# baggepinnen/LPVSpectral.jl

Hardware: NVIDIA B200
Metric: windowed LS spectra/sec (higher is better)
Workload: dtype f64

## Files before the change

### lpvspectral.jl_b200/csrc/api.cu

```cuda
#include <math.h>
#include <stdarg.h>
#include <stdlib.h>
#include <stdio.h>
#include <string.h>

#include <algorithm>

#include "ctx.h"

namespace lpvs {

int fail(lpvs_ctx* c, int code, const char* fmt, ...) {
    char buf[512];
    va_list ap;
    va_start(ap, fmt);
    vsnprintf(buf, sizeof buf, fmt, ap);
    va_end(ap);
    if (c) c->err = buf;
    return code;
}

void* ws_raw(lpvs_ctx* c, int slot, size_t bytes) {
    DevBuf& b = c->buf[slot];
    if (bytes == 0) bytes = 16;
// ... 140 lines not shown
    if (i >= count) return;
    double s = accumulate ? out[i] : 0.0;
    for (int p = 0; p < nparts; p++) s += parts[(long long)p * stride + i];
    out[i] = s;
}

__global__ void k_check_finite(const double* __restrict__ v, long long n, int* flag) {
    bool bad = false;
    for (long long i = (long long)blockIdx.x * blockDim.x + threadIdx.x; i < n; i += (long long)gridDim.x * blockDim.x)
        bad |= !isfinite(v[i]);
    if (bad) atomicOr(flag, 1);
}

__global__ void k_first_nonfinite_channel(const double* __restrict__ Y, long long ldY, long long N, int* out) {
    const int ch = blockIdx.y;
    bool bad = false;
    for (long long i = (long long)blockIdx.x * blockDim.x + threadIdx.x; i < N; i += (long long)gridDim.x * blockDim.x)
        bad |= !isfinite(Y[ch * ldY + i]);
    if (bad) atomicMin(out, ch);
}

__global__ void k_jitter_ridge(const double* __restrict__ maxdiag, double ridge, double scale, double* __restrict__ out) {
    out[0] = fmax(ridge, scale * maxdiag[0]);
}

__global__ void k_merge_windows(const double* __restrict__ pieces, long long K, int n, int hop, long long N,
                                double* __restrict__ out) {
    const long long s = (long long)blockIdx.x * blockDim.x + threadIdx.x;
    if (s >= N) return;
    long long k0 = s >= n ? (s - n + hop) / hop : 0;
    long long k1 = s / hop;
    if (k1 > K - 1) k1 = K - 1;
    double acc = 0.0;
    long long cnt = 0;
    for (long long k = k0; k <= k1; k++) {
        acc += pieces[k * n + (s - k * hop)];
        cnt++;
    }
    out[s] = acc / (double)(cnt > 0 ? cnt : 1);
}

__global__ void k_x_to_complex(const double* __restrict__ X, int Np, int Nf, int zero_first, int nrhs,
                               double* __restrict__ out) {
    int k = blockIdx.x * blockDim.x + threadIdx.x;
    if (k >= Nf) return;
    int pc = (k >> 6) * 128 + (k & 63);
    for (int r = 0; r < nrhs; r++) {
        double re = X[(long long)r * Np + pc];
        double im = (zero_first && k == 0) ? 0.0 : X[(long long)r * Np + pc + 64];
        out[((long long)r * Nf + k) * 2] = re;
        out[((long long)r * Nf + k) * 2 + 1] = im;
    }
}

__device__ __forceinline__ int ref_to_internal(int j, int Nf, int zero_first) {
    if (j < Nf) return (j >> 6) * 128 + (j & 63);
    int k = j - Nf + zero_first;
    return (k >> 6) * 128 + 64 + (k & 63);
}
__global__ void k_gather_ref(const double* __restrict__ G, const double* __restrict__ B, int Np, int Nf,
                             int zero_first, int Nreg, double* __restrict__ Gout, double* __restrict__ bout) {
    int j = blockIdx.x * blockDim.x + threadIdx.x;
    int i = blockIdx.y;
    if (j >= Nreg) return;
    int pi = ref_to_internal(i, Nf, zero_first), pj = ref_to_internal(j, Nf, zero_first);
    int a = max(pi, pj), b = min(pi, pj);
    double v = G[(long long)a * Np + b];
    Gout[(long long)i * Nreg + j] = v;
    if (bout && i == 0) bout[j] = B[pj];
}
__global__ void k_scatter_ref_vec(const double* __restrict__ xin, int Nf, int zero_first, int Nreg, int Np,
                                  double* __restrict__ xout) {
    int p = blockIdx.x * blockDim.x + threadIdx.x;
    if (p >= Np) return;
    int q = p >> 7, r = p & 127, part = r >> 6, cc = q * 64 + (r & 63);
    double v = 0.0;
    if (cc < Nf && !(zero_first && part == 1 && cc == 0)) {
        int j = part == 0 ? cc : (Nf + cc - zero_first);
        v = xin[j];
    }
    xout[p] = v;
}

__global__ void k_window_accum(int kind, const double* __restrict__ X, long long strideB, int Np, int nwin, int Nf,
                               int zero_first, double* __restrict__ sums) {
    int k = blockIdx.x * blockDim.x + threadIdx.x;
    if (k >= Nf) return;
    int pc = (k >> 6) * 128 + (k & 63);
    bool noim = zero_first && k == 0;
    if (kind == LPVS_WIN_PSD) {
        double s = sums[k];
        for (int wdx = 0; wdx < nwin; wdx++) {
            const double* x = X + (long long)wdx * strideB;
            double re = x[pc], im = noim ? 0.0 : x[pc + 64];
            s = __dadd_rn(s, __dadd_rn(__dmul_rn(re, re), __dmul_rn(im, im)));
        }
        sums[k] = s;
    } else if (kind == LPVS_WIN_CSD) {
        double sr = sums[k], si = sums[Nf + k];
        for (int wdx = 0; wdx < nwin; wdx++) {
            const double* x = X + (long long)wdx * strideB;
            double ar = x[pc], ai = noim ? 0.0 : x[pc + 64];
            double br = x[Np + pc], bi = noim ? 0.0 : x[Np + pc + 64];
            sr = __dadd_rn(sr, __dadd_rn(__dmul_rn(ar, br), __dmul_rn(ai, bi)));
            si = __dadd_rn(si, __dsub_rn(__dmul_rn(ai, br), __dmul_rn(ar, bi)));
        }
        sums[k] = sr;
        sums[Nf + k] = si;
    } else {
        double syy = sums[k], suu = sums[Nf + k], sr = sums[2 * Nf + k], si = sums[3 * Nf + k];
        for (int wdx = 0; wdx < nwin; wdx++) {
            const double* x = X + (long long)wdx * strideB;
            double ar = x[pc], ai = noim ? 0.0 : x[pc + 64];
            double br = x[Np + pc], bi = noim ? 0.0 : x[Np + pc + 64];
            sr = __dadd_rn(sr, __dadd_rn(__dmul_rn(ar, br), __dmul_rn(ai, bi)));
            si = __dadd_rn(si, __dsub_rn(__dmul_rn(ai, br), __dmul_rn(ar, bi)));
            syy = __dadd_rn(syy, __dadd_rn(__dmul_rn(ar, ar), __dmul_rn(ai, ai)));
            suu = __dadd_rn(suu, __dadd_rn(__dmul_rn(br, br), __dmul_rn(bi, bi)));
        }
        sums[k] = syy;
        sums[Nf + k] = suu;
        sums[2 * Nf + k] = sr;
        sums[3 * Nf + k] = si;
    }
}

__global__ void k_window_matrix_accum(const double* __restrict__ X, long long strideB, int Np, int C, int nwin, int Nf,
                                      int zero_first, double* __restrict__ sums) {
    const long long idx = (long long)blockIdx.x * blockDim.x + threadIdx.x;
    if (idx >= (long long)Nf * C * C) return;
    const int k = (int)(idx / ((long long)C * C)), i = (int)(idx / C % C), j = (int)(idx % C);
    if (i > j) return;
    const int pc = (k >> 6) * 128 + (k & 63);
    const bool noim = zero_first && k == 0;
    double* sij = sums + 2 * (((long long)k * C + i) * C + j);
    double sr = sij[0], si = sij[1];
    for (int wdx = 0; wdx < nwin; wdx++) {
        const double* xi = X + (long long)wdx * strideB + (long long)i * Np;
        const double* xj = X + (long long)wdx * strideB + (long long)j * Np;
        const double ar = xi[pc], ai = noim ? 0.0 : xi[pc + 64];
        const double br = xj[pc], bi = noim ? 0.0 : xj[pc + 64];
        sr = __dadd_rn(sr, __dadd_rn(__dmul_rn(ar, br), __dmul_rn(ai, bi)));
        si = __dadd_rn(si, __dsub_rn(__dmul_rn(ai, br), __dmul_rn(ar, bi)));
    }
    sij[0] = sr;
    sij[1] = si;
    if (i != j) {
        double* sji = sums + 2 * (((long long)k * C + j) * C + i);
        sji[0] = sr;
        sji[1] = -si;
    }
}

void fill_basis_args(const FourierPlan& pl, GramArgs& g) {
    g.ncc = pl.Nf;
    g.nblk = pl.nblk;
    g.f = pl.d_f;
    g.wtab = pl.d_wtab;
    g.gscale = pl.dd * pl.dd;
    g.bscale = pl.dd;
    g.E = nullptr;
    g.Kt = nullptr;
    g.lpv_nf = 1;
}

static int structured_sums(lpvs_ctx* c, const FourierPlan& pl, const StructuredLayout& lay, const GramArgs& g, int nprob,
                           double2* Z) {
    double2* tab = ws<double2>(c, BUF_SANC, (size_t)lay.nrows * g.tbl_ns);
    if (!tab) return fail(c, LPVS_E_NOMEM, "out of device memory (sum tables)");
    launch_sum_tables(g.t, g.tbl_base, g.tbl_ns, pl.d_sfreq, lay.nzb, structured_layout(pl.f0, pl.Nf, 2).nzb, tab, c->st);
    SumArgs a{};
    a.t = g.t;
    a.W = g.W;
    a.y = g.y;
    a.u = g.u;
    a.w_abs = g.w_abs;
    a.start0 = g.start0;
    a.hop = g.hop;
    a.n = g.n;
    a.s_end = g.s_end;
    a.tab = tab;
    a.tbl_base = g.tbl_base;
    a.tbl_ns = g.tbl_ns;
    a.nzg = lay.nzg;
    a.nby = lay.nby;
    a.nzb = lay.nzb;
    a.Z = Z;
    a.strideZ = (long long)lay.nzb * FB;
    c->launches += 1 + launch_trig_sums(a, nprob, c->st);
    return LPVS_OK;
}
static void structured_fill(lpvs_ctx* c, const FourierPlan& pl, const StructuredLayout& lay, const double2* Z, double* G,
                            long long strideG, double* B, long long strideB, int nrhs, int nprob) {
    FillArgs fa{};
    fa.Z = Z;
    fa.strideZ = (long long)lay.nzb * FB;
    fa.zm_off = lay.zm_off;
    fa.zp_off = lay.zp_off;
    fa.zy_off[0] = lay.zy_off[0];
    fa.zy_off[1] = lay.zy_off[1];
    fa.ncc = pl.Nf;
    fa.nblk = pl.nblk;
    fa.zero_first = pl.zero_first;
    fa.gscale = pl.dd * pl.dd;
    fa.G = G;
    fa.strideG = strideG;
    c->launches += launch_gram_fill(fa, nprob, c->st);
// ... 383 lines not shown
        case LPVS_OPT_ADMM_SYMV: c->admm_symv = (int)value; break;
        case LPVS_OPT_TRSV_FLOW: c->trsv_flow = (int)value != 0; break;
        case LPVS_OPT_ADMM_M32: c->admm_m32 = (int)value != 0; break;
        case LPVS_OPT_SHARD_EXCHANGE:
            if ((int)value < 0 || (int)value > 2) return fail(c, LPVS_E_BAD_ARG, "LPVS_OPT_SHARD_EXCHANGE must be 0, 1 or 2");
            c->shard_exchange = (int)value;
            break;
        default: return fail(c, LPVS_E_BAD_ARG, "unknown option %d", key);
    }
    return LPVS_OK;
}

int lpvs_set_stream(lpvs_ctx* c, void* stream) {
    if (!c) return LPVS_E_BAD_ARG;
    Lock lk(c->mu);
    cudaSetDevice(c->device);
    cudaStreamSynchronize(c->st);
    c->st = stream ? (cudaStream_t)stream : c->own_st;
    return LPVS_OK;
}

int64_t lpvs_launch_count(const lpvs_ctx* c) { return c ? c->launches : 0; }

int lpvs_last_gram_timing(const lpvs_ctx* c, double* ms, int64_t* launches, double* flops) {
    if (!c) return LPVS_E_BAD_ARG;
    if (ms) *ms = c->gram_ms;
    if (launches) *launches = c->gram_launches;
    if (flops) *flops = c->gram_flops;
    return LPVS_OK;
}

int lpvs_last_call_ms(const lpvs_ctx* c, double* ms) {
    if (!c || !ms) return LPVS_E_BAD_ARG;
    float m = 0.f;
    if (cudaEventSynchronize(c->ev_call1) != cudaSuccess || cudaEventElapsedTime(&m, c->ev_call0, c->ev_call1) != cudaSuccess) {
        cudaGetLastError();
        return LPVS_E_CUDA;
    }
    *ms = m;
    return LPVS_OK;
}

int lpvs_dev_alloc(lpvs_ctx* c, int64_t bytes, void** dptr) {
    if (!c || !dptr) return LPVS_E_BAD_ARG;
    cudaSetDevice(c->device);
    LPVS_CU(c, cudaMalloc(dptr, (size_t)bytes));
    return LPVS_OK;
}
int lpvs_dev_free(lpvs_ctx* c, void* dptr) {
    if (!c) return LPVS_E_BAD_ARG;
    cudaSetDevice(c->device);
    cudaStreamSynchronize(c->st);
    LPVS_CU(c, cudaFree(dptr));
    return LPVS_OK;
}
int lpvs_dev_upload(lpvs_ctx* c, void* dptr, const void* hptr, int64_t bytes) {
    if (!c) return LPVS_E_BAD_ARG;
    cudaSetDevice(c->device);
    LPVS_CU(c, cudaMemcpyAsync(dptr, hptr, (size_t)bytes, cudaMemcpyHostToDevice, c->st));
    LPVS_CU(c, cudaStreamSynchronize(c->st));
    return LPVS_OK;
}
int lpvs_dev_download(lpvs_ctx* c, void* hptr, const void* dptr, int64_t bytes) {
    if (!c) return LPVS_E_BAD_ARG;
    cudaSetDevice(c->device);
    LPVS_CU(c, cudaMemcpyAsync(hptr, dptr, (size_t)bytes, cudaMemcpyDeviceToHost, c->st));
    LPVS_CU(c, cudaStreamSynchronize(c->st));
    return LPVS_OK;
}
int lpvs_release_workspace(lpvs_ctx* c) {
    if (!c) return LPVS_E_BAD_ARG;
    Lock lk(c->mu);
    cudaSetDevice(c->device);
    LPVS_CU(c, cudaStreamSynchronize(c->st));
    for (auto& b : c->buf) {
        if (b.p) cudaFree(b.p);
        b.p = nullptr;
        b.cap = 0;
    }
    return LPVS_OK;
}
int lpvs_sync(lpvs_ctx* c) {
    if (!c) return LPVS_E_BAD_ARG;
    LPVS_CU(c, cudaStreamSynchronize(c->st));
    return LPVS_OK;
}

int64_t lpvs_window_count(int64_t N, int n, int noverlap) {
    if (n <= 0) return 0;
    if (noverlap < 0) noverlap = n >> 1;
    if (noverlap >= n) return -1;
    return N >= n ? (N - n) / (n - noverlap) + 1 : 0;
}

int lpvs_gram_fourier(lpvs_ctx* c, const double* y, const double* t, int64_t N, const double* f, int Nf,
                      const double* W, double* G, double* b) {
    if (!c) return LPVS_E_BAD_ARG;
    Lock lk(c->mu);
    CallTimer call_timer(c);
    cudaSetDevice(c->device);
    if (!t || N <= 0 || !G) return fail(c, LPVS_E_BAD_ARG, "bad arguments");
    gram_timer_reset(c);
    FourierPlan pl;
    int rc = make_fourier_plan(c, f, Nf, &pl);
    if (rc) return rc;
    double *d_t, *d_y, *d_W;
    if ((rc = upload(c, BUF_T, t, N, &d_t))) return rc;
    if ((rc = upload(c, BUF_Y, y, N, &d_y))) return rc;
    if ((rc = upload(c, BUF_W, W, N, &d_W))) return rc;
    const long long Np = pl.Np;
    double* d_G = ws<double>(c, BUF_G, (size_t)Np * Np);
    double* d_B = ws<double>(c, BUF_B, (size_t)2 * Np);
    if (!d_G || !d_B) return fail(c, LPVS_E_NOMEM, "out of device memory (G)");
    if ((rc = gram_single(c, pl, d_t, d_y, nullptr, d_W, N, y ? 1 : 0, d_G, d_B))) return rc;
    double* d_out = ws<double>(c, BUF_MISC, (size_t)pl.Nreg * pl.Nreg + pl.Nreg);
    if (!d_out) return fail(c, LPVS_E_NOMEM, "out of device memory (G out)");
    dim3 grid((pl.Nreg + 127) / 128, pl.Nreg);
    k_gather_ref<<<grid, 128, 0, c->st>>>(d_G, (y && b) ? d_B : nullptr, pl.Np, pl.Nf, pl.zero_first, pl.Nreg, d_out,
                                          (y && b) ? d_out + (size_t)pl.Nreg * pl.Nreg : nullptr);
    c->launches++;
    LPVS_CU(c, cudaMemcpyAsync(G, d_out, sizeof(double) * pl.Nreg * pl.Nreg, cudaMemcpyDeviceToHost, c->st));
    if (y && b)
        LPVS_CU(c, cudaMemcpyAsync(b, d_out + (size_t)pl.Nreg * pl.Nreg, sizeof(double) * pl.Nreg,
                                   cudaMemcpyDeviceToHost, c->st));
    LPVS_CU(c, cudaStreamSynchronize(c->st));
    gram_timer_resolve(c);
    return LPVS_OK;
}

}

namespace lpvs {
int ls_solve_dev(lpvs_ctx* c, const FourierPlan& pl, const double* d_t, const double* d_y, const double* d_u,
                        const double* d_W, int64_t N, int nrhs, double ridge, bool allow_jitter, double** d_x,
                        int* info) {
    const long long Np = pl.Np;
    double* d_G = ws<double>(c, BUF_G, (size_t)Np * Np);
    double* d_B = ws<double>(c, BUF_B, (size_t)2 * Np);
    double* d_md = ws<double>(c, BUF_SUMS, 8);
    if (!d_G || !d_B || !d_md) return fail(c, LPVS_E_NOMEM, "out of device memory (G)");
    int rc;
    if (info) *info = 0;
    if (!d_W && nrhs == 1 && allow_jitter) {
        auto regram = [&]() { return gram_single(c, pl, d_t, d_y, nullptr, nullptr, N, 1, d_G, d_B); };
        if ((rc = regram())) return rc;
        OpArgs op;
        op.mode = GRAM_DIRECT;
        op.t = d_t;
        op.f = pl.d_f;
        op.dd = pl.dd;
        op.ncc = pl.Nf;
        op.zero_first = pl.zero_first;
        op.N = N;
        if ((rc = ls_solve_accurate(c, op, pl.Np, pl.zero_first, d_y, d_G, d_B, sqrt(ridge), regram, info))) return rc;
        *d_x = d_B;
        return LPVS_OK;
    }
    double* d_keep = nullptr;
    for (int attempt = 0; attempt < 2; attempt++) {
        if (attempt == 0) {
            if ((rc = gram_single(c, pl, d_t, d_y, d_u, d_W, N, nrhs, d_G, d_B))) return rc;
            if (allow_jitter) {
                d_keep = ws<double>(c, BUF_YINV, (size_t)Np * Np + 2 * Np);
                if (d_keep) {
                    LPVS_CU(c, cudaMemcpyAsync(d_keep, d_G, sizeof(double) * Np * Np, cudaMemcpyDeviceToDevice, c->st));
                    LPVS_CU(c, cudaMemcpyAsync(d_keep + Np * Np, d_B, sizeof(double) * 2 * Np, cudaMemcpyDeviceToDevice,
// ... 318 lines not shown
        double* d_G = ws<double>(c, BUF_G, (size_t)nw * Np * Np);
        double* d_B = ws<double>(c, BUF_B, (size_t)nw * 2 * Np);
        if (!d_G || !d_B) return fail(c, LPVS_E_NOMEM, "out of device memory (window batch of %d)", nw);
        GramArgs g{};
        fill_basis_args(pl, g);
        auto chain_tables = [&]() -> int {
            double2* anc = ws<double2>(c, BUF_ANC, (size_t)pl.ngroups * ns);
            double2* del = ws<double2>(c, BUF_DEL, (size_t)ns);
            if (!anc || !del) return fail(c, LPVS_E_NOMEM, "out of device memory (anchor table)");
            launch_anchor_table(d_t, s0, ns, pl.d_f, pl.nblk, pl.df, anc, del, c->st);
            c->launches++;
            g.anc = anc;
            g.del = del;
            return LPVS_OK;
        };
        if (gram_is_chain(pl.mode) && !pl.structured && (rc = chain_tables())) return rc;
        g.t = d_t;
        g.y = d_y;
        g.u = nrhs > 1 ? d_u : nullptr;
        g.W = d_W;
        g.w_abs = 0;
        g.start0 = s0;
        g.hop = hop;
        g.n = n;
        g.s_end = N;
        g.nrhs = nrhs;
        g.tbl_base = s0;
        g.tbl_ns = ns;
        g.G = d_G;
        g.strideG = Np * Np;
        g.B = d_B;
        g.strideB = 2 * Np;
        gram_timer_begin(c);
        if (pl.structured) {
            const StructuredLayout lay = structured_layout(pl.f0, Nf, nrhs);
            double2* Z = ws<double2>(c, BUF_ZSUM, (size_t)nw * lay.nzb * FB);
            if (!Z) return fail(c, LPVS_E_NOMEM, "out of device memory (window sums)");
            if ((rc = structured_sums(c, pl, lay, g, nw, Z))) return rc;
            structured_fill(c, pl, lay, Z, d_G, Np * Np, d_B, 2 * Np, nrhs, nw);
            if (pl.structured_ref && (rc = structured_correct(c, pl, g, d_G, Np * Np, d_B, 2 * Np, nrhs, nw, k_begin * hop,
                                                              (k_end - 1 - k_begin) * hop + n)))
                return rc;
            gram_timer_end(c, (double)nw * n * lay.nzb * FB * 8.0, 1);
        } else {
            c->launches += launch_gram(pl.mode, g, nw, c->st);
            gram_timer_end(c, (double)nw * n * pl.Nreg * (pl.Nreg + 1.0), 1);
        }
        if ((rc = factor_solve(c, pl.Nf, pl.zero_first, pl.Np, d_G, d_B, nrhs, lambda, nw, hinfo.data()))) return rc;
        LPVS_CU(c, cudaStreamSynchronize(c->st));
        for (int i = 0; i < nw; i++) {
            if (!hinfo[i]) continue;
            if (!c->jitter) {
                if (!bad) {
                    bad = hinfo[i];
                    bad_window = k0 + i;
                }
                continue;
            }
            double* d_g1 = ws<double>(c, BUF_YINV, (size_t)Np * Np + 2 * Np + 8);
            if (!d_g1) return fail(c, LPVS_E_NOMEM, "out of device memory (window retry)");
            double* d_b1 = d_g1 + Np * Np;
            double* d_md = d_b1 + 2 * Np;
            if (pl.structured && !g.anc && (rc = chain_tables())) return rc;
            GramArgs g1 = g;
            g1.start0 = g.start0 + (long long)i * hop;
            g1.G = d_g1;
            g1.B = d_b1;
            c->launches += launch_gram(pl.mode, g1, 1, c->st);
            launch_max_diag(d_g1, Np * Np, pl.Np, pl.Nf, pl.zero_first, d_md, 1, c->st);
            k_jitter_ridge<<<1, 1, 0, c->st>>>(d_md, lambda, (double)pl.Nreg * 2.220446049250313e-16, d_md + 1);
            c->launches += 2;
            int pinfo = 0;
            if ((rc = factor_solve(c, pl.Nf, pl.zero_first, pl.Np, d_g1, d_b1, nrhs, 0.0, 1, &pinfo, nullptr, 0.0, d_md + 1)))
                return rc;
            LPVS_CU(c, cudaMemcpyAsync(d_B + (long long)i * 2 * Np, d_b1, sizeof(double) * 2 * Np, cudaMemcpyDeviceToDevice,
                                       c->st));
            LPVS_CU(c, cudaStreamSynchronize(c->st));
            if (pinfo && !bad) {
                bad = pinfo;
                bad_window = k0 + i;
            }
            jittered++;
        }
        k_window_accum<<<(Nf + 127) / 128, 128, 0, c->st>>>(kind, d_B, 2 * Np, pl.Np, nw, Nf, pl.zero_first, d_sums);
        c->launches++;
    }
    LPVS_CU(c, cudaMemcpyAsync(sums, d_sums, sizeof(double) * slen, cudaMemcpyDeviceToHost, c->st));
    LPVS_CU(c, cudaStreamSynchronize(c->st));
    gram_timer_resolve(c);
    if (bad) {
        if (info) *info = bad;
        return fail(c, LPVS_E_NOT_SPD, "Cholesky breakdown in window %lld at internal pivot %d",
                    (long long)(c->window_base + bad_window), bad);
    }
    if (jittered && info) *info = LPVS_INFO_JITTER;
    return LPVS_OK;
}

int lpvs_ls_window_sums(lpvs_ctx* c, int kind, const double* y, const double* u, const double* t, int64_t N,
                        const double* f, int Nf, const double* W, int n, int noverlap, double lambda, int64_t k_begin,
                        int64_t k_end, double* sums, int* info) {
    if (!c) return LPVS_E_BAD_ARG;
    Lock lk(c->mu);
    CallTimer call_timer(c);
    if (!y || !t || N <= 0 || n <= 0) return fail(c, LPVS_E_BAD_ARG, "bad arguments");
    if (noverlap < 0) noverlap = n >> 1;
    if (noverlap >= n) return fail(c, LPVS_E_BAD_ARG, "noverlap must be < n");
    cudaSetDevice(c->device);
    const int64_t K = lpvs_window_count(N, n, noverlap);
    if (k_begin < 0 || k_end > K || k_begin > k_end) return fail(c, LPVS_E_BAD_ARG, "window range out of bounds");
    if (k_end == k_begin) {
        if (sums) memset(sums, 0, sizeof(double) * sums_len(kind, Nf));
        return LPVS_OK;
    }
    double *d_t, *d_y, *d_u;
    int rc;
    const int64_t hop = n - noverlap, s0 = k_begin * hop, s1 = (k_end - 1) * hop + n;
    if ((rc = upload(c, BUF_T, t + s0, s1 - s0, &d_t))) return rc;
    if ((rc = upload(c, BUF_Y, y + s0, s1 - s0, &d_y))) return rc;
    if ((rc = upload(c, BUF_U, u ? u + s0 : nullptr, s1 - s0, &d_u))) return rc;
    c->window_base = k_begin;
    int rc2 = lpvs_ls_window_sums_dev(c, kind, d_y, d_u, d_t, s1 - s0, f, Nf, W, n, noverlap, lambda, 0,
                                      k_end - k_begin, sums, info);
    c->window_base = 0;
    int rcf = inputs_finite(c);
    return rcf ? rcf : rc2;
}

int lpvs_ls_window_matrix_sums_dev(lpvs_ctx* c, const double* d_Y, int C, int64_t ldY, const double* d_t, int64_t N,
                                   const double* f, int Nf, const double* W, int n, int noverlap, double lambda,
                                   int64_t k_begin, int64_t k_end, double* sums, int* info) {
    if (!c) return LPVS_E_BAD_ARG;
    Lock lk(c->mu);
    CallTimer call_timer(c);
    cudaSetDevice(c->device);
    if (info) *info = 0;
    if (C < 1) return fail(c, LPVS_E_BAD_ARG, "C must be >= 1 (got %d)", C);
    if (ldY < N) return fail(c, LPVS_E_BAD_ARG, "ldY (%lld) must be >= N (%lld)", (long long)ldY, (long long)N);
    if (!d_Y || !d_t || !W || !sums || n <= 0 || Nf <= 0) return fail(c, LPVS_E_BAD_ARG, "bad arguments");
    if (noverlap < 0) noverlap = n >> 1;
    if (noverlap >= n) return fail(c, LPVS_E_BAD_ARG, "noverlap must be < n");
    const int64_t K = lpvs_window_count(N, n, noverlap);
    if (k_begin < 0 || k_end > K || k_begin > k_end) return fail(c, LPVS_E_BAD_ARG, "window range out of bounds");
    gram_timer_reset(c);
    FourierPlan pl;
    int rc = make_fourier_plan(c, f, Nf, &pl);
    if (rc) return rc;
    const long long slen = 2LL * Nf * C * C;
    double* d_sums = ws<double>(c, BUF_SUMS, (size_t)slen);
    double* d_W;
    if ((rc = upload(c, BUF_W, W, n, &d_W))) return rc;
    if (!d_sums) return fail(c, LPVS_E_NOMEM, "out of device memory (%lld sums)", slen);
    LPVS_CU(c, cudaMemsetAsync(d_sums, 0, sizeof(double) * slen, c->st));
    const long long Np = pl.Np, hop = n - noverlap;
    const int nb = pl.Np / TB;
    const long long per_win = (Np * Np + Np * TB + (long long)C * Np) * 8;
    int64_t batch = c->window_batch > 0 ? c->window_batch : std::max<int64_t>(1, (6LL << 30) / per_win);
    if (c->window_batch <= 0 && batch > c->sms) batch -= batch % c->sms;
    batch = std::min<int64_t>(std::min<int64_t>(batch, 32768), std::max<int64_t>(1, k_end - k_begin));
    std::vector<int> hinfo((size_t)batch);
    int bad = 0, jittered = 0;
    int64_t bad_window = -1;
    for (int64_t k0 = k_begin; k0 < k_end; k0 += batch) {
        const int nw = (int)std::min<int64_t>(batch, k_end - k0);
        const long long s0 = k0 * hop, ns = (long long)(nw - 1) * hop + n;
        double* d_G = ws<double>(c, BUF_G, (size_t)nw * Np * Np);
        double* d_B = ws<double>(c, BUF_B, (size_t)nw * C * Np);
// ... 224 lines not shown
    auto cleanup = [&]() { cudaStreamSynchronize(c->st); };
    for (int64_t k0 = 0; k0 < nwin && !bad; k0 += batch) {
        const int nw = (int)std::min<int64_t>(batch, nwin - k0);
        const long long s0 = k0 * hop, ns = (long long)(nw - 1) * hop + n;
        double* d_G = ws<double>(c, BUF_G, (size_t)nw * Np * Np);
        double* d_Y = ws<double>(c, BUF_YINV, (size_t)nw * Np * Np);
        double* d_B = ws<double>(c, BUF_B, (size_t)nw * 2 * Np);
        if (!d_G || !d_Y || !d_B) {
            cleanup();
            return fail(c, LPVS_E_NOMEM, "out of device memory (window batch of %d)", nw);
        }
        GramArgs g{};
        fill_basis_args(pl, g);
        if (gram_is_chain(pl.mode) && !pl.structured) {
            double2* anc = ws<double2>(c, BUF_ANC, (size_t)pl.ngroups * ns);
            double2* del = ws<double2>(c, BUF_DEL, (size_t)ns);
            if (!anc || !del) {
                cleanup();
                return fail(c, LPVS_E_NOMEM, "out of device memory (anchor table)");
            }
            launch_anchor_table(d_t, s0, ns, pl.d_f, pl.nblk, pl.df, anc, del, c->st);
            c->launches++;
            g.anc = anc;
            g.del = del;
        }
        g.t = d_t;
        g.y = d_y;
        g.u = nrhs > 1 ? d_u : nullptr;
        g.W = d_W;
        g.w_abs = 0;
        g.start0 = s0;
        g.hop = hop;
        g.n = n;
        g.s_end = Nloc;
        g.nrhs = nrhs;
        g.tbl_base = s0;
        g.tbl_ns = ns;
        g.G = d_G;
        g.strideG = Np * Np;
        g.B = d_B;
        g.strideB = 2 * Np;
        gram_timer_begin(c);
        if (pl.structured) {
            const StructuredLayout lay = structured_layout(pl.f0, Nf, nrhs);
            double2* Z = ws<double2>(c, BUF_ZSUM, (size_t)nw * lay.nzb * FB);
            if (!Z || (rc = structured_sums(c, pl, lay, g, nw, Z))) {
                cleanup();
                return Z ? rc : fail(c, LPVS_E_NOMEM, "out of device memory (window sums)");
            }
            structured_fill(c, pl, lay, Z, d_G, Np * Np, d_B, 2 * Np, nrhs, nw);
            if (pl.structured_ref && (rc = structured_correct(c, pl, g, d_G, Np * Np, d_B, 2 * Np, nrhs, nw))) {
                cleanup();
                return rc;
            }
            gram_timer_end(c, (double)nw * n * lay.nzb * FB * 8.0, 1);
        } else {
            c->launches += launch_gram(pl.mode, g, nw, c->st);
            gram_timer_end(c, (double)nw * n * pl.Nreg * (pl.Nreg + 1.0), 1);
        }
        CholArgs ca{};
        ca.G = d_G;
        ca.strideG = Np * Np;
        ca.Y = d_Y;
        ca.strideY = Np * Np;
        ca.Linv = ws<double>(c, BUF_LINV, (size_t)nw * nb * TB * TB);
        ca.strideLinv = (long long)nb * TB * TB;
        ca.info = ws<int>(c, BUF_INFO, (size_t)nw);
        ca.Np = pl.Np;
        ca.nb = nb;
        if (!ca.Linv || !ca.info) {
            cleanup();
            return fail(c, LPVS_E_NOMEM, "out of device memory (factor workspace)");
        }
        cudaMemsetAsync(ca.info, 0, sizeof(int) * nw, c->st);
        launch_diag_prepare(d_G, ca.strideG, pl.Np, pl.Nf, pl.zero_first, nullptr, 1.0 / mu, nw, c->st);
        c->launches += 1 + potrf(ca, nw, c->sms, c->st);
        c->launches += potri(ca, nw, c->st);
        cudaMemcpyAsync(hinfo.data(), ca.info, sizeof(int) * nw, cudaMemcpyDeviceToHost, c->st);
        if ((rc = admm_batch_run(c, d_G, d_B, pl.Np, nrhs, nw, prox_kind, prox_param, mu, 1, iters, tol, d_its,
                                 d_res, pl.Nf, pl.zero_first))) {
            cleanup();
            return rc;
        }
        k_window_accum<<<(Nf + 127) / 128, 128, 0, c->st>>>(kind, d_B, 2 * Np, pl.Np, nw, Nf, pl.zero_first, d_sums);
        c->launches++;
        if (iters_done)
            cudaMemcpyAsync(hits.data(), d_its, sizeof(long long) * nw * nrhs, cudaMemcpyDeviceToHost, c->st);
        if (residuals)
            cudaMemcpyAsync(residuals + k0 * nrhs, d_res, sizeof(double) * nw * nrhs, cudaMemcpyDeviceToHost, c->st);
        cudaError_t e = cudaStreamSynchronize(c->st);
        if (e != cudaSuccess) {
            cleanup();
            return fail(c, LPVS_E_CUDA, "windowed sparse batch failed: %s", cudaGetErrorString(e));
        }
        if (iters_done)
            for (int i = 0; i < nw * nrhs; i++) iters_done[k0 * nrhs + i] = hits[i];
        for (int i = 0; i < nw && !bad; i++)
            if (hinfo[i]) {
                bad = hinfo[i];
                bad_window = k_begin + k0 + i;
            }
    }
    cleanup();
    if ((rc = inputs_finite(c))) return rc;
    if (bad) {
        if (info) *info = bad;
        return fail(c, LPVS_E_NOT_SPD, "Cholesky breakdown in window %lld at internal pivot %d", (long long)bad_window,
                    bad);
    }
    LPVS_CU(c, cudaMemcpyAsync(sums, d_sums, sizeof(double) * slen, cudaMemcpyDeviceToHost, c->st));
    LPVS_CU(c, cudaStreamSynchronize(c->st));
    gram_timer_resolve(c);
    return LPVS_OK;
}

static int window_matrix_sparse_check(lpvs_ctx* c, int C, int64_t ldY, int64_t N, int n, int noverlap, int prox_kind,
                                      double mu, int64_t k_begin, int64_t k_end) {
    if (C < 1) return fail(c, LPVS_E_BAD_ARG, "C must be >= 1 (got %d)", C);
    if (ldY < N) return fail(c, LPVS_E_BAD_ARG, "ldY (%lld) must be >= N (%lld)", (long long)ldY, (long long)N);
    if (N <= 0 || n <= 0) return fail(c, LPVS_E_BAD_ARG, "bad arguments");
    if (!(mu > 0.0) || mu > 1.0) return fail(c, LPVS_E_BAD_ARG, "mu should be in (0, 1]");
    if (prox_kind < LPVS_PROX_L1 || prox_kind > LPVS_PROX_BALL_L0)
        return fail(c, LPVS_E_BAD_ARG, "prox kind %d not valid for the Fourier problem", prox_kind);
    if (noverlap >= n) return fail(c, LPVS_E_BAD_ARG, "noverlap must be < n");
    const int64_t K = lpvs_window_count(N, n, noverlap < 0 ? n >> 1 : noverlap);
    if (k_begin < 0 || k_end > K || k_begin > k_end) return fail(c, LPVS_E_BAD_ARG, "window range out of bounds");
    return LPVS_OK;
}

int lpvs_ls_window_matrix_sparse_sums_dev(lpvs_ctx* c, const double* d_Y, int C, int64_t ldY, const double* d_t,
                                          int64_t N, const double* f, int Nf, const double* W, int n, int noverlap,
                                          int prox_kind, double prox_param, double mu, int64_t iters, double tol,
                                          int64_t k_begin, int64_t k_end, double* sums, int64_t* iters_done,
                                          double* residuals, int* info) {
    if (!c) return LPVS_E_BAD_ARG;
    Lock lk(c->mu);
    CallTimer call_timer(c);
    cudaSetDevice(c->device);
    if (info) *info = 0;
    int rc = window_matrix_sparse_check(c, C, ldY, N, n, noverlap, prox_kind, mu, k_begin, k_end);
    if (rc) return rc;
    if (!d_Y || !d_t || !W || !sums || Nf <= 0) return fail(c, LPVS_E_BAD_ARG, "bad arguments");
    if (C > 65535) return fail(c, LPVS_E_UNSUPPORTED, "C = %d channels: at most 65535", C);
    if (noverlap < 0) noverlap = n >> 1;
    const long long slen = 2LL * Nf * C * C;
    if (k_end == k_begin) {
        memset(sums, 0, sizeof(double) * slen);
        return LPVS_OK;
    }
    gram_timer_reset(c);
    FourierPlan pl;
    if ((rc = make_fourier_plan(c, f, Nf, &pl))) return rc;
    double* d_sums = ws<double>(c, BUF_SUMS, (size_t)slen);
    double* d_W;
    if ((rc = upload(c, BUF_W, W, n, &d_W))) return rc;
    if (!d_sums) return fail(c, LPVS_E_NOMEM, "out of device memory (%lld sums)", slen);
    LPVS_CU(c, cudaMemsetAsync(d_sums, 0, sizeof(double) * slen, c->st));
    const long long Np = pl.Np, hop = n - noverlap;
    const int nb = pl.Np / TB;
    const long long per_win = (2 * Np * Np + Np * TB + 8LL * C * Np) * 8;
    int64_t batch = c->window_batch > 0 ? c->window_batch : std::max<int64_t>(1, (6LL << 30) / per_win);
    if (c->window_batch <= 0 && batch > c->sms) batch -= batch % c->sms;
    batch = std::min<int64_t>(std::min<int64_t>(batch, 32768), k_end - k_begin);
    std::vector<int> hinfo((size_t)batch);
    std::vector<long long> hits((size_t)batch * C);
    long long* d_its = ws<long long>(c, BUF_WIN_ITS, (size_t)batch * C);
    double* d_res = ws<double>(c, BUF_WIN_RES, (size_t)batch * C);
// ... 201 lines not shown
```

Measured before the change: 24680.

## Pipeline window accumulation through shared memory with multi-stage cp.async

Rewrites the per-frequency window accumulation kernel so each block handles 32 frequencies and stages chunks of 32 windows into shared memory with a 4-stage cp.async pipeline. Only 32 of the 128 threads compute sums, while all threads cooperate on loads. The goal is more blocks for small Nf and latency hiding on the strided per-window global reads. In exchange, 96 threads per block sit idle during compute, and there is a per-call cudaGetDevice plus extra shared memory per block. It also adds an internal test entry point for the kernel.

```diff
diff --git a/lpvspectral.jl_b200/csrc/api.cu b/lpvspectral.jl_b200/csrc/api.cu
--- a/lpvspectral.jl_b200/csrc/api.cu
+++ b/lpvspectral.jl_b200/csrc/api.cu
@@ -246,47 +246,92 @@
     xout[p] = v;
 }
 
-__global__ void k_window_accum(int kind, const double* __restrict__ X, long long strideB, int Np, int nwin, int Nf,
-                               int zero_first, double* __restrict__ sums) {
-    int k = blockIdx.x * blockDim.x + threadIdx.x;
-    if (k >= Nf) return;
-    int pc = (k >> 6) * 128 + (k & 63);
-    bool noim = zero_first && k == 0;
-    if (kind == LPVS_WIN_PSD) {
-        double s = sums[k];
-        for (int wdx = 0; wdx < nwin; wdx++) {
-            const double* x = X + (long long)wdx * strideB;
-            double re = x[pc], im = noim ? 0.0 : x[pc + 64];
-            s = __dadd_rn(s, __dadd_rn(__dmul_rn(re, re), __dmul_rn(im, im)));
-        }
-        sums[k] = s;
-    } else if (kind == LPVS_WIN_CSD) {
-        double sr = sums[k], si = sums[Nf + k];
-        for (int wdx = 0; wdx < nwin; wdx++) {
-            const double* x = X + (long long)wdx * strideB;
-            double ar = x[pc], ai = noim ? 0.0 : x[pc + 64];
-            double br = x[Np + pc], bi = noim ? 0.0 : x[Np + pc + 64];
-            sr = __dadd_rn(sr, __dadd_rn(__dmul_rn(ar, br), __dmul_rn(ai, bi)));
-            si = __dadd_rn(si, __dsub_rn(__dmul_rn(ai, br), __dmul_rn(ar, bi)));
-        }
-        sums[k] = sr;
-        sums[Nf + k] = si;
-    } else {
-        double syy = sums[k], suu = sums[Nf + k], sr = sums[2 * Nf + k], si = sums[3 * Nf + k];
-        for (int wdx = 0; wdx < nwin; wdx++) {
-            const double* x = X + (long long)wdx * strideB;
-            double ar = x[pc], ai = noim ? 0.0 : x[pc + 64];
-            double br = x[Np + pc], bi = noim ? 0.0 : x[Np + pc + 64];
-            sr = __dadd_rn(sr, __dadd_rn(__dmul_rn(ar, br), __dmul_rn(ai, bi)));
-            si = __dadd_rn(si, __dsub_rn(__dmul_rn(ai, br), __dmul_rn(ar, bi)));
-            syy = __dadd_rn(syy, __dadd_rn(__dmul_rn(ar, ar), __dmul_rn(ai, ai)));
-            suu = __dadd_rn(suu, __dadd_rn(__dmul_rn(br, br), __dmul_rn(bi, bi)));
-        }
-        sums[k] = syy;
-        sums[Nf + k] = suu;
-        sums[2 * Nf + k] = sr;
-        sums[3 * Nf + k] = si;
-    }
+constexpr int WA_F = 32, WA_W = 32, WA_S = 4, WA_T = 128;
+constexpr size_t WA_SMEM_MAX = sizeof(double) * WA_S * WA_W * 4 * WA_F;
+
+__global__ void __launch_bounds__(WA_T) k_window_accum(int kind, const double* __restrict__ X, long long strideB, int Np,
+                                                       int nwin, int Nf, int zero_first, double* __restrict__ sums) {
+    extern __shared__ __align__(16) double wbuf[];
+    const int nvec = kind == LPVS_WIN_PSD ? 2 : 4;
+    const int k0 = blockIdx.x * WA_F, pc0 = (k0 >> 6) * 128 + (k0 & 63), tid = threadIdx.x;
+    const int stage_d = WA_W * nvec * WA_F, nchunk = (nwin + WA_W - 1) / WA_W;
+    auto issue = [&](int ch) {
+        if (ch < nchunk) {
+            double* dst = wbuf + (ch % WA_S) * stage_d;
+            const int w0 = ch * WA_W, nw = min(WA_W, nwin - w0);
+            for (int e = tid; e < nw * nvec * (WA_F / 2); e += WA_T) {
+                const int seg = e % (WA_F / 2), v = e / (WA_F / 2) % nvec, w = e / (nvec * (WA_F / 2));
+                cp_async16(dst + (w * nvec + v) * WA_F + 2 * seg,
+                           X + (long long)(w0 + w) * strideB + (v >> 1) * Np + pc0 + (v & 1) * 64 + 2 * seg);
+            }
+        }
+        cp_async_commit();
+    };
+    const int k = k0 + tid;
+    const bool sum_lane = tid < WA_F && k < Nf, noim = zero_first && k == 0;
+    double s0 = 0.0, s1 = 0.0, s2 = 0.0, s3 = 0.0;
+    if (sum_lane) {
+        s0 = sums[k];
+        if (kind != LPVS_WIN_PSD) s1 = sums[Nf + k];
+        if (kind == LPVS_WIN_COHERE) {
+            s2 = sums[2 * Nf + k];
+            s3 = sums[3 * Nf + k];
+        }
+    }
+#pragma unroll
+    for (int s = 0; s < WA_S - 1; s++) issue(s);
+    for (int ch = 0; ch < nchunk; ch++) {
+        issue(ch + WA_S - 1);
+        cp_async_wait<WA_S - 1>();
+        __syncthreads();
+        if (sum_lane) {
+            const double* x = wbuf + (ch % WA_S) * stage_d + tid;
+            const int nw = min(WA_W, nwin - ch * WA_W);
+            if (kind == LPVS_WIN_PSD) {
+                for (int w = 0; w < nw; w++, x += 2 * WA_F) {
+                    const double re = x[0], im = noim ? 0.0 : x[WA_F];
+                    s0 = __dadd_rn(s0, __dadd_rn(__dmul_rn(re, re), __dmul_rn(im, im)));
+                }
+            } else {
+                for (int w = 0; w < nw; w++, x += 4 * WA_F) {
+                    const double ar = x[0], ai = noim ? 0.0 : x[WA_F];
+                    const double br = x[2 * WA_F], bi = noim ? 0.0 : x[3 * WA_F];
+                    if (kind == LPVS_WIN_CSD) {
+                        s0 = __dadd_rn(s0, __dadd_rn(__dmul_rn(ar, br), __dmul_rn(ai, bi)));
+                        s1 = __dadd_rn(s1, __dsub_rn(__dmul_rn(ai, br), __dmul_rn(ar, bi)));
+                    } else {
+                        s2 = __dadd_rn(s2, __dadd_rn(__dmul_rn(ar, br), __dmul_rn(ai, bi)));
+                        s3 = __dadd_rn(s3, __dsub_rn(__dmul_rn(ai, br), __dmul_rn(ar, bi)));
+                        s0 = __dadd_rn(s0, __dadd_rn(__dmul_rn(ar, ar), __dmul_rn(ai, ai)));
+                        s1 = __dadd_rn(s1, __dadd_rn(__dmul_rn(br, br), __dmul_rn(bi, bi)));
+                    }
+                }
+            }
+        }
+        __syncthreads();
+    }
+    cp_async_wait<0>();
+    if (sum_lane) {
+        sums[k] = s0;
+        if (kind != LPVS_WIN_PSD) sums[Nf + k] = s1;
+        if (kind == LPVS_WIN_COHERE) {
+            sums[2 * Nf + k] = s2;
+            sums[3 * Nf + k] = s3;
+        }
+    }
+}
+
+void launch_window_accum(int kind, const double* X, long long strideB, int Np, int nwin, int Nf, int zero_first,
+                         double* sums, cudaStream_t st) {
+    static bool attr_done[64] = {};
+    int dev = 0;
+    cudaGetDevice(&dev);
+    if (!attr_done[dev & 63]) {
+        cudaFuncSetAttribute(k_window_accum, cudaFuncAttributeMaxDynamicSharedMemorySize, (int)WA_SMEM_MAX);
+        attr_done[dev & 63] = true;
+    }
+    const size_t smem = sizeof(double) * WA_S * WA_W * (kind == LPVS_WIN_PSD ? 2 : 4) * WA_F;
+    k_window_accum<<<(Nf + WA_F - 1) / WA_F, WA_T, smem, st>>>(kind, X, strideB, Np, nwin, Nf, zero_first, sums);
 }
 
 __global__ void k_window_matrix_accum(const double* __restrict__ X, long long strideB, int Np, int C, int nwin, int Nf,
@@ -836,6 +881,18 @@
 }
 int lpvs_sync(lpvs_ctx* c) {
     if (!c) return LPVS_E_BAD_ARG;
+    LPVS_CU(c, cudaStreamSynchronize(c->st));
+    return LPVS_OK;
+}
+
+int lpvs_internal_window_accum(lpvs_ctx* c, int kind, const double* d_X, int64_t strideB, int Np, int64_t nwin, int Nf,
+                               int zero_first, double* d_sums) {
+    if (!c) return LPVS_E_BAD_ARG;
+    if (kind < LPVS_WIN_PSD || kind > LPVS_WIN_COHERE || Nf <= 0 || Np != 128 * ((Nf + 63) / 64) || nwin < 0 ||
+        nwin > INT32_MAX || strideB < (kind == LPVS_WIN_PSD ? 1 : 2) * (int64_t)Np || strideB % 2 || (!d_X && nwin > 0) || !d_sums)
+        return fail(c, LPVS_E_BAD_ARG, "lpvs_internal_window_accum: bad arguments");
+    launch_window_accum(kind, d_X, strideB, Np, (int)nwin, Nf, zero_first ? 1 : 0, d_sums, c->st);
+    LPVS_CU(c, cudaGetLastError());
     LPVS_CU(c, cudaStreamSynchronize(c->st));
     return LPVS_OK;
 }
@@ -1320,7 +1377,7 @@
             }
             jittered++;
         }
-        k_window_accum<<<(Nf + 127) / 128, 128, 0, c->st>>>(kind, d_B, 2 * Np, pl.Np, nw, Nf, pl.zero_first, d_sums);
+        launch_window_accum(kind, d_B, 2 * Np, pl.Np, nw, Nf, pl.zero_first, d_sums, c->st);
         c->launches++;
     }
     LPVS_CU(c, cudaMemcpyAsync(sums, d_sums, sizeof(double) * slen, cudaMemcpyDeviceToHost, c->st));
@@ -1711,7 +1768,7 @@
             cleanup();
             return rc;
         }
-        k_window_accum<<<(Nf + 127) / 128, 128, 0, c->st>>>(kind, d_B, 2 * Np, pl.Np, nw, Nf, pl.zero_first, d_sums);
+        launch_window_accum(kind, d_B, 2 * Np, pl.Np, nw, Nf, pl.zero_first, d_sums, c->st);
         c->launches++;
         if (iters_done)
             cudaMemcpyAsync(hits.data(), d_its, sizeof(long long) * nw * nrhs, cudaMemcpyDeviceToHost, c->st);
```

After: 24760, median of 6. No clear change (+0.3%).
